# davek44/Glimmer-MG

Hardware: AMD Instinct MI355X
Metric: Mbases/s scored (6-frame IMM) (higher is better)
Workload: dtype f64

## Files before the change

glimmer-mg_amd/csrc/gmg_api.hip:

```cpp

#include "gmg_internal.h"
#include "gmg_scan.h"

#include <ctype.h>
#include <stdarg.h>
#include <stdio.h>
#include <stdlib.h>
#include <string.h>
#include <new>
#include <mutex>
#include <vector>

static thread_local char g_err[512] = "";
static int g_device = -1;

int gmg_set_error(int code, const char *fmt, ...)
{
    va_list ap;
    va_start(ap, fmt);
    vsnprintf(g_err, sizeof g_err, fmt, ap);
    va_end(ap);
    return code;
}

extern "C" const char *gmg_last_error(void) { return g_err; }

long long g_gmg_opt[GMG_OPT_COUNT] = {
     0,  0,  0,  0,  0,  0,
     0,  -1,  0x7ffffffell,  0,  0,
     0,  0,  1,  1,  1,  1,  2,
     -1,  0,  1,  1,  0,  4,  0,  64ll << 20,  0,  0};
static const char *const g_opt_name[GMG_OPT_COUNT] = {
    "seg_plain", "mg_tile", "mg_one_stream", "mg_err_flat", "mg_err_calls", "mg_err_calls_grow", "orfs_exact_path",
    "train_sort_min", "mg_max_entries", "mg_timing", "ingest_timing", "train_timing", "diag", "strings_fused",
    "mg_gene32", "mg_fused", "mg_err_skip", "mg_orfs_events", "mg_err_tile", "mg_err_tile_q", "mg_err_qonly", "mg_err_wave", "mg_err_wave_q", "orfs_walk8", "ingest_scans", "ingest_piece_min", "mg_orfs_bits", "orfs_q_poison"};

static int opt_index(const char *key)
{
    for (int i = 0; key && i < GMG_OPT_COUNT; i++)
        if (strcmp(key, g_opt_name[i]) == 0) return i;
    return -1;
}

extern "C" int gmg_set_option(const char *key, long long value)
{
    const int i = opt_index(key);
    if (i < 0) return gmg_set_error(GMG_EINVAL, "gmg_set_option: unknown option '%s'", key ? key : "(null)");
#ifndef GMG_ABLATIONS
    if (i == GMG_OPT_DIAG && value != 0)
        return gmg_set_error(GMG_EINVAL, "gmg_set_option: the ablation kernels are not in this build (-DGMG_ABLATIONS)");
#endif
    if (i == GMG_OPT_MG_MAX_ENTRIES && (value < 1 || value > 0x7ffffffell))
        return gmg_set_error(GMG_EINVAL, "gmg_set_option: mg_max_entries must be in [1, 2^31 - 2]");
    g_gmg_opt[i] = value;
    return GMG_OK;
}

extern "C" int gmg_get_option(const char *key, long long *value)
{
    const int i = opt_index(key);
    if (i < 0 || !value) return gmg_set_error(GMG_EINVAL, "gmg_get_option: unknown option '%s'", key ? key : "(null)");
    *value = g_gmg_opt[i];
    return GMG_OK;
}

static void options_from_env(void)
{
    for (int i = 0; i < GMG_OPT_COUNT; i++) {
        char name[64] = "GMG_";
        size_t k = 4;
        for (const char *c = g_opt_name[i]; *c && k + 1 < sizeof name; c++) name[k++] = (char)toupper((unsigned char)*c);
        name[k] = 0;
        const char *v = getenv(name);
        if (!v) continue;
        char *end = nullptr;
        long long x = strtoll(v, &end, 10);
        if (end == v) x = 1;
        (void)gmg_set_option(g_opt_name[i], x);
    }
}
extern "C" const char *gmg_version(void) { return "glimmer-mg_amd 0.1 (gfx950)"; }

extern "C" int gmg_device_count(void)
{
    int n = 0;
    if (hipGetDeviceCount(&n) != hipSuccess) return 0;
    return n;
}

extern "C" int gmg_init(int device)
{
    int n = 0;
    hipError_t e = hipGetDeviceCount(&n);
    if (e != hipSuccess || n <= 0)
        return gmg_set_error(GMG_ENODEV, "gmg_init: no HIP device (%s); there is no CPU fallback",
                             e == hipSuccess ? "count = 0" : hipGetErrorString(e));
    if (device < 0 || device >= n)
        return gmg_set_error(GMG_EINVAL, "gmg_init: device %d out of range (have %d)", device, n);
    hipDeviceProp_t prop;
    GMG_HIP(hipGetDeviceProperties(&prop, device));
    if (strncmp(prop.gcnArchName, "gfx950", 6) != 0)
        return gmg_set_error(GMG_ENODEV, "gmg_init: device %d is %s; this library is built for gfx950 only",
                             device, prop.gcnArchName);
    GMG_HIP(hipSetDevice(device));
    if (g_device < 0) options_from_env();
    g_device = device;
    return GMG_OK;
}

int gmg_enter(const char *who)
{
    if (g_device < 0) return gmg_set_error(GMG_ENODEV, "%s: gmg_init() has not succeeded in this process", who);
    int cur = -1;
    if (hipGetDevice(&cur) != hipSuccess || cur != g_device) GMG_HIP(hipSetDevice(g_device));
    return GMG_OK;
}

static int require_init(const char *who) { return gmg_enter(who); }

extern "C" int gmg_synchronize(void *stream)
{
    int rc = gmg_enter("gmg_synchronize");
    if (rc) return rc;
    GMG_HIP(hipStreamSynchronize((hipStream_t)stream));
    return GMG_OK;
}


extern "C" int gmg_base_code(int ch)
{
    switch (tolower(ch & 0xff)) {
    case 'a': return 0;
    case 'c': return 1;
    case 'g': case 'r': case 'd': return 2;
    case 't': case 'w': case 'k': return 3;
    default: return 1;
    }
}

extern "C" uint64_t gmg_packed_words(uint64_t total_bases) { return (total_bases + 15) / 16 + 1; }

static const uint8_t *base_code_table(void)
{
    static const struct Table {
        uint8_t code[256];
        Table() { for (int c = 0; c < 256; c++) code[c] = (uint8_t)gmg_base_code(c); }
    } table;
    return table.code;
}

extern "C" int gmg_pack_bases(const char *ascii, uint64_t n, uint64_t first_base, uint32_t *packed)
{
    if ((!ascii && n) || !packed) return gmg_set_error(GMG_EINVAL, "gmg_pack_bases: NULL argument");
    const uint8_t *code = base_code_table();
    const unsigned char *a = (const unsigned char *)ascii;
    uint64_t i = 0, g = first_base;
    for (; i < n && (g & 15); i++, g++) packed[g >> 4] |= (uint32_t)code[a[i]] << (2 * (g & 15));
    for (; i + 16 <= n; i += 16, g += 16) {
        uint32_t w = 0;
        for (int k = 0; k < 16; k++) w |= (uint32_t)code[a[i + k]] << (2 * k);
        packed[g >> 4] |= w;
    }
    for (; i < n; i++, g++) packed[g >> 4] |= (uint32_t)code[a[i]] << (2 * (g & 15));
    return GMG_OK;
}


static inline int parent_of(int x) { return (x - 1) / 4; }

static int final_row(const int16_t *mip, int n) { return mip[n] == -2 ? parent_of(n) : n; }

static void complete_tree(const int16_t *mip, const float *prob, int D, uint8_t *cshift, float *crow)
{
    std::vector<int> cur(1, 0), nxt;
    size_t lvl_base = 0, lvl_size = 1;
    for (int l = 0; l <= D; l++) {
        if (l < D) nxt.assign(lvl_size * 4, 0);
        for (size_t i = 0; i < lvl_size; i++) {
            int st = cur[i];
            int row = (st >= 0) ? final_row(mip, st) : ~st;
            memcpy(crow + 4 * (lvl_base + i), prob + 4 * (size_t)row, 4 * sizeof(float));
            if (l == D) continue;
            uint8_t sh = 0;
            if (st >= 0 && mip[st] >= 0) {
                sh = (uint8_t)(2 * mip[st]);
                for (int b = 0; b < 4; b++) nxt[4 * i + b] = 4 * st + 1 + b;
            } else {
                for (int b = 0; b < 4; b++) nxt[4 * i + b] = ~row;
            }
            cshift[lvl_base + i] = sh;
        }
        lvl_base += lvl_size;
        lvl_size *= 4;
        cur.swap(nxt);
    }
}

static float dense_entry(const int16_t *mip, const float *prob, int W, int D, uint32_t idx)
{
    int node = 0;
    for (int i = 0; i < D; i++) {
        int pos = mip[node];
        if (pos == -1) break;
        if (pos < -1) { node = parent_of(node); break; }
        node = 4 * node + (int)((idx >> (2 * pos)) & 3) + 1;
    }
    if (mip[node] < -1) node = parent_of(node);
    return prob[4 * (size_t)node + ((idx >> (2 * (W - 1))) & 3)];
}

static float dense_part_entry(const int16_t *mip, const float *prob, int W, int D, int j, uint32_t idx)
{
    int node = 0, start = j - (W - 1);
    for (int i = 0; i < D; i++) {
        int q = start + mip[node];
        if (q < 0) break;
        node = 4 * node + (int)((idx >> (2 * q)) & 3) + 1;
    }
    if (mip[node] == -2) node = parent_of(node);
    return prob[4 * (size_t)node + ((idx >> (2 * j)) & 3)];
}

static size_t align_up(size_t x, size_t a) { return (x + a - 1) / a * a; }

extern "C" int gmg_model_upload(const int16_t *mip, const float *prob4, int W, int D, int P, int N,
                                gmg_model **out)
{
    int rc = require_init("gmg_model_upload");
    if (rc) return rc;
    if (!mip || !prob4 || !out) return gmg_set_error(GMG_EINVAL, "gmg_model_upload: NULL argument");
    if (W < 1 || W > GMG_MAX_MODEL_LEN || D < 0 || D > 12 || P < 1 || N < 1)
        return gmg_set_error(GMG_EBADMODEL, "gmg_model_upload: unsupported shape len=%d depth=%d period=%d nodes=%d",
                             W, D, P, N);
    long need = 0, pw = 1;
    for (int l = 0; l <= D; l++) { need += pw; pw *= 4; }
    if (N < need)
        return gmg_set_error(GMG_EBADMODEL, "gmg_model_upload: num_nodes=%d < %ld needed for depth %d", N, need, D);
    const size_t PN = (size_t)P * N;
    for (size_t i = 0; i < PN; i++)
        if (mip[i] < -2 || mip[i] > W - 1)
            return gmg_set_error(GMG_EBADMODEL, "gmg_model_upload: mut_info_pos %d at slot %zu outside [-2,%d]",
                                 (int)mip[i], i, W - 1);

    const bool fast = (W <= GMG_FAST_MAX_LEN && D <= GMG_FAST_MAX_DEPTH);
    const bool dense = (W <= GMG_DENSE_MAX_LEN);
    const size_t n_internal = (size_t)((pw / 4 - 1) / 3);
    const size_t ctot = (size_t)need;
    const size_t cstride = align_up(n_internal ? n_internal : 1, 16);
    const size_t n_dense = dense ? ((size_t)1 << (2 * W)) : 0;
    const size_t n_part = dense ? (n_dense - 4) / 3 : 0;

    size_t o_mip = 0;
    size_t o_prob = align_up(o_mip + PN, 256);
    size_t o_cshift = align_up(o_prob + PN * 16, 256);
    size_t o_crow = align_up(o_cshift + (fast ? P * cstride : 0), 256);
    size_t o_chalf = align_up(o_crow + (fast ? (size_t)P * ctot * 16 + 16 : 0), 256);
    const size_t n_leaves = (size_t)(pw / 4);
    size_t o_dense = align_up(o_chalf + (fast ? (size_t)P * n_leaves * 16 : 0), 256);
    size_t o_part = align_up(o_dense + (size_t)P * n_dense * 4, 256);
    size_t total = align_up(o_part + (size_t)P * n_part * 4 + 4, 256);

    std::vector<unsigned char> blob(total, 0);
    int8_t *h_mip = (int8_t *)(blob.data() + o_mip);
    for (size_t i = 0; i < PN; i++) h_mip[i] = (int8_t)mip[i];
    memcpy(blob.data() + o_prob, prob4, PN * 16);
    if (fast)
        for (int p = 0; p < P; p++)
            complete_tree(mip + (size_t)p * N, prob4 + 4 * (size_t)p * N, D,
                          blob.data() + o_cshift + p * cstride,
                          (float *)(blob.data() + o_crow) + (size_t)p * ctot * 4);
    if (fast)
        for (int p = 0; p < P; p++) {
            const float *leaf = (const float *)(blob.data() + o_crow) + ((size_t)p * ctot + n_internal) * 4;
            float *half = (float *)(blob.data() + o_chalf) + (size_t)p * n_leaves * 4;
            for (size_t r = 0; r < n_leaves; r++)
                for (int h = 0; h < 2; h++) {
                    half[(h * n_leaves + r) * 2] = leaf[4 * r + 2 * h];
                    half[(h * n_leaves + r) * 2 + 1] = leaf[4 * r + 2 * h + 1];
                }
        }
    if (dense)
        for (int p = 0; p < P; p++) {
            const int16_t *pm = mip + (size_t)p * N;
            const float *pp = prob4 + 4 * (size_t)p * N;
            float *full = (float *)(blob.data() + o_dense) + (size_t)p * n_dense;
            float *part = (float *)(blob.data() + o_part) + (size_t)p * n_part;
            for (uint32_t idx = 0; idx < n_dense; idx++) full[idx] = dense_entry(pm, pp, W, D, idx);
            size_t o = 0;
            for (int j = 0; j < W - 1; j++) {
                uint32_t cnt = 1u << (2 * (j + 1));
                for (uint32_t idx = 0; idx < cnt; idx++) part[o + idx] = dense_part_entry(pm, pp, W, D, j, idx);
                o += cnt;
            }
        }

    gmg_model *m = new (std::nothrow) gmg_model();
    if (!m) return gmg_set_error(GMG_ENOMEM, "gmg_model_upload: out of host memory");
    hipError_t e = hipMalloc(&m->d_blob, total);
    if (e != hipSuccess) { delete m; return gmg_set_error(GMG_ENOMEM, "gmg_model_upload: hipMalloc(%zu): %s", total, hipGetErrorString(e)); }
    e = hipMemcpy(m->d_blob, blob.data(), total, hipMemcpyHostToDevice);
    if (e != hipSuccess) { (void)hipFree(m->d_blob); delete m; return gmg_set_error(GMG_EHIP, "gmg_model_upload: hipMemcpy: %s", hipGetErrorString(e)); }
    m->blob_bytes = total;
    m->min_exp = 255;
    m->max_exp = 0;
    m->odd_values = 0;
    for (size_t i = 0; i < PN * 4; i++) {
        uint32_t b;
        memcpy(&b, &prob4[i], 4);
        const uint32_t ex = (b >> 23) & 0xffu;
        if (mip[i >> 2] == -2) continue;
        if ((b << 1) == 0) continue;
        if ((b >> 31) == 0 || ex == 0 || ex == 255) m->odd_values = 1;
        if ((int)ex < m->min_exp) m->min_exp = (int)ex;
        if ((int)ex > m->max_exp) m->max_exp = (int)ex;
    }
    unsigned char *d = (unsigned char *)m->d_blob;
    m->dev.W = W; m->dev.D = D; m->dev.P = P; m->dev.N = N;
    m->dev.mip = (const int8_t *)(d + o_mip);
    m->dev.prob = (const float *)(d + o_prob);
    m->dev.cshift = fast ? (const uint8_t *)(d + o_cshift) : nullptr;
    m->dev.crow = fast ? (const float *)(d + o_crow) : nullptr;
    m->dev.chalf = fast ? (const float *)(d + o_chalf) : nullptr;
    m->dev.cstride = (int)cstride;
    m->dev.ctot = (int)ctot;
    m->dev.has_fast = fast;
    m->dev.dense = dense ? (const float *)(d + o_dense) : nullptr;
    m->dev.dense_part = dense ? (const float *)(d + o_part) : nullptr;
    m->dev.n_dense_part = (int)n_part;
    m->dev.has_dense = dense;
    *out = m;
    return GMG_OK;
}

extern "C" int gmg_model_free(gmg_model *m)
{
    if (!m) return GMG_OK;
    if (m->d_blob) (void)hipFree(m->d_blob);
    delete m;
    return GMG_OK;
}

extern "C" int gmg_model_info(const gmg_model *m, int *W, int *D, int *P, int *N)
{
    if (!m) return gmg_set_error(GMG_EINVAL, "gmg_model_info: NULL model");
    if (W) *W = m->dev.W;
    if (D) *D = m->dev.D;
    if (P) *P = m->dev.P;
    if (N) *N = m->dev.N;
    return GMG_OK;
}

extern "C" int gmg_null_set_upload(const gmg_model *const *models, int n, gmg_null_set **out)
{
    int rc = require_init("gmg_null_set_upload");
    if (rc) return rc;
    if (!models || n < 1 || !out) return gmg_set_error(GMG_EINVAL, "gmg_null_set_upload: bad argument");
    for (int i = 0; i < n; i++)
        if (!models[i] || !models[i]->dev.has_dense || models[i]->dev.W != 3 || models[i]->dev.P != 3)
            return gmg_set_error(GMG_EBADMODEL, "gmg_null_set_upload: model %d is not a (3,2,3) Build_Indep_WO_Stops model", i);
    gmg_null_set *ns = new (std::nothrow) gmg_null_set();
    if (!ns) return gmg_set_error(GMG_ENOMEM, "gmg_null_set_upload: out of host memory");
    ns->d_tab = nullptr;
    ns->n = n;
    ns->min_exp = 255; ns->max_exp = 0; ns->odd_values = 0;
    for (int i = 0; i < n; i++) {
        if (models[i]->min_exp < ns->min_exp) ns->min_exp = models[i]->min_exp;
        if (models[i]->max_exp > ns->max_exp) ns->max_exp = models[i]->max_exp;
        ns->odd_values |= models[i]->odd_values;
    }
    hipError_t e = hipMalloc((void **)&ns->d_tab, (size_t)n * 252 * sizeof(float));
    for (int i = 0; i < n && e == hipSuccess; i++) {
        e = hipMemcpy(ns->d_tab + (size_t)i * 252, models[i]->dev.dense, 192 * sizeof(float), hipMemcpyDeviceToDevice);
        if (e == hipSuccess) e = hipMemcpy(ns->d_tab + (size_t)i * 252 + 192, models[i]->dev.dense_part, 60 * sizeof(float), hipMemcpyDeviceToDevice);
    }
    if (e != hipSuccess) { gmg_null_set_free(ns); return gmg_set_error(GMG_EHIP, "gmg_null_set_upload: %s", hipGetErrorString(e)); }
    *out = ns;
    return GMG_OK;
}

extern "C" int gmg_null_set_from_tables(const int16_t *mip, const float *prob4, int n, gmg_null_set **out)
{
    int rc = require_init("gmg_null_set_from_tables");
    if (rc) return rc;
    if (!mip || !prob4 || n < 1 || !out) return gmg_set_error(GMG_EINVAL, "gmg_null_set_from_tables: bad argument");
    for (size_t i = 0; i < (size_t)n * 63; i++)
        if (mip[i] < -2 || mip[i] > 2)
            return gmg_set_error(GMG_EBADMODEL, "gmg_null_set_from_tables: mut_info_pos %d in model %zu outside [-2,2]", (int)mip[i], i / 63);
    gmg_null_set *ns = new (std::nothrow) gmg_null_set();
    if (!ns) return gmg_set_error(GMG_ENOMEM, "gmg_null_set_from_tables: out of host memory");
    ns->d_tab = nullptr;
    ns->n = n;
    ns->min_exp = 255; ns->max_exp = 0; ns->odd_values = 0;
    std::vector<float> tab((size_t)n * 252);
    for (int i = 0; i < n; i++)
        for (int p = 0; p < 3; p++) {
            const int16_t *pm = mip + ((size_t)i * 3 + p) * 21;
            const float *pp = prob4 + ((size_t)i * 3 + p) * 21 * 4;
            float *full = tab.data() + (size_t)i * 252 + p * 64, *part = tab.data() + (size_t)i * 252 + 192 + p * 20;
            for (uint32_t idx = 0; idx < 64; idx++) full[idx] = dense_entry(pm, pp, 3, 2, idx);
            size_t o = 0;
            for (int j = 0; j < 2; j++) {
                const uint32_t cnt = 1u << (2 * (j + 1));
                for (uint32_t idx = 0; idx < cnt; idx++) part[o + idx] = dense_part_entry(pm, pp, 3, 2, j, idx);
                o += cnt;
            }
            for (int k = 0; k < 21 * 4; k++) {
                uint32_t b;
                memcpy(&b, pp + k, 4);
// ... 759 lines not shown
```

glimmer-mg_amd/csrc/gmg_frame6.hip:

```cpp

#include "gmg_device.h"
#include <stdlib.h>
#include <vector>

#ifndef GMG_F6_STAMPS
#define GMG_F6_STAMPS 0
#endif
#if GMG_F6_STAMPS
__device__ unsigned long long g_f6_stamps[1024 * 16 * 8];
extern "C" int gmg_debug_f6_stamps(unsigned long long *out, int n)
{
    return hipMemcpyFromSymbol(out, HIP_SYMBOL(g_f6_stamps), (size_t)n * 8) == hipSuccess ? 0 : -1;
}
#define F6_STAMP(i) do { const unsigned long long now_ = __builtin_readcyclecounter(); st_acc[i] += now_ - st_prev; st_prev = now_; } while (0)
#else
#define F6_STAMP(i) do { } while (0)
#endif

struct Frame6Args {
    GmgDevModel gene, nul;
    const uint32_t *packed;
    const uint64_t *off;
    const uint32_t *tile_read;
    uint64_t total, n_reads;
// ... 380 lines not shown
                        const double nf = s_nf[__builtin_amdgcn_ubfe(mt, mb + 4 + 2 * b, 6)];
                        const double nr = s_nr[__builtin_amdgcn_ubfe(mt, mb + 2 * b, 6)];
                        v[2 * b] = (double)gf - nf;
                        v[2 * b + 1] = (double)gr - nr;
                    }
                }
                const uint64_t chunk = MULTI ? round_chunk0 + (uint64_t)k : chunk0 + (uint64_t)(j0 + k) * chunk_step;
                if (SUM) {
                    sum_chunk((uint32_t)k, v);
                } else if (GENE_ONLY) {
                    float *gf = a.out_gene + (uint64_t)(STRINGS ? 1 : ftype) * a.gstride + chunk * SPAN;
                    float *gr = a.out_gene + (uint64_t)(STRINGS ? 0 : 3 + ftype) * a.gstride + chunk * SPAN;
                    if (PAIR) {
                        typedef float f2 __attribute__((ext_vector_type(2)));
                        const f2 x0 = {(float)v[0], (float)v[2]}, x1 = {(float)v[1], (float)v[3]};
                        __builtin_nontemporal_store(x0, (f2 *)(gf + lane_off));
                        __builtin_nontemporal_store(x1, (f2 *)(gr + lane_off));
                    } else {
                        gf[lane_off] = (float)v[0]; gf[lane_off + 1] = (float)v[2];
                        gr[lane_off] = (float)v[1]; gr[lane_off + 1] = (float)v[3];
                    }
                } else if (DIAG & 1) {
                    if (v[0] + v[1] + v[2] + v[3] == 1.2345e300) a.out[lane_off] = v[0];
                } else {
                    double *pf = out_f + chunk * SPAN, *pr = out_r + chunk * SPAN;
                    if (PAIR) {
                        typedef double d2 __attribute__((ext_vector_type(2)));
                        const d2 x0 = {v[0], v[2]}, x1 = {v[1], v[3]};
                        __builtin_nontemporal_store(x0, (d2 *)(pf + lane_off));
                        __builtin_nontemporal_store(x1, (d2 *)(pr + lane_off));
                    } else {
                        __builtin_nontemporal_store(v[0], pf + lane_off);
                        __builtin_nontemporal_store(v[2], pf + lane_off + 1);
                        __builtin_nontemporal_store(v[1], pr + lane_off);
                        __builtin_nontemporal_store(v[3], pr + lane_off + 1);
                    }
                }
            }
        }
        if (SUM) {
            __syncthreads();
            round_flush();
        }
        F6_STAMP(4);
    }
#if GMG_F6_STAMPS
    if ((threadIdx.x & 63u) == 0 && blockIdx.x < 1024)
        for (int i = 0; i < 8; i++) g_f6_stamps[(blockIdx.x * 16 + (threadIdx.x >> 6)) * 8 + i] = st_acc[i];
#endif
}


__device__ __forceinline__ void f6_generic_range(const Frame6Args &a, const GmgDevModel &gene, uint64_t first, uint64_t count,
                                                 uint64_t i0, uint64_t n_lanes)
{
    for (uint64_t i = i0; i < count; i += n_lanes) {
        const uint64_t g = first + i;
        uint64_t r = a.tile_read[g / GMG_TILE];
        uint64_t r_end = a.off[r + 1];
        while (g >= r_end) { r++; r_end = a.off[r + 1]; }
        const uint64_t r_off = a.off[r];
        const int L = (int)(r_end - r_off);
        const int p = (int)(g - r_off);
        DevBuf bf = dev_make_buf(a.packed, r_off, 0, (uint32_t)L, GMG_REVERSED);
        DevBuf br = dev_make_buf(a.packed, r_off, 0, (uint32_t)L, GMG_COMPLEMENTED);
        for (int f = 0; f < 3; f++) {
            if (a.out_gene) {
                a.out_gene[(uint64_t)f * a.gstride + g] = dev_score(gene, bf, L - 1 - p, f);
                a.out_gene[(uint64_t)(3 + f) * a.gstride + g] = dev_score(gene, br, p, f);
                continue;
            }
            a.out[(uint64_t)f * a.stride + g] =
                (double)dev_score(gene, bf, L - 1 - p, f) - (double)dev_score(a.nul, bf, L - 1 - p, f);
            a.out[(uint64_t)(3 + f) * a.stride + g] =
                (double)dev_score(gene, br, p, f) - (double)dev_score(a.nul, br, p, f);
        }
    }
}
__device__ __forceinline__ void f6_generic_range(const Frame6Args &a, uint64_t i0, uint64_t n_lanes)
{
    f6_generic_range(a, a.gene, a.first, a.count, i0, n_lanes);
}

template <int DT, int U, bool GENE = false, bool MULTI = false>
__global__ __launch_bounds__(256) void k_frame6p(Frame6Args a)
{
    extern __shared__ __attribute__((aligned(16))) uint8_t s_shift[];
    if (MULTI) {
        if (blockIdx.x < 8 * a.n_ranges) {
            const F6Range rg = a.ranges[blockIdx.x / 8];
            f6_generic_range(a, a.gmodels[rg.group], rg.first, rg.count, (uint64_t)(blockIdx.x % 8) * blockDim.x + threadIdx.x, (uint64_t)8 * blockDim.x);
            return;
        }
    } else if (blockIdx.x >= a.p_blocks) {
        f6_generic_range(a, (uint64_t)(blockIdx.x - a.p_blocks) * blockDim.x + threadIdx.x, (uint64_t)(gridDim.x - a.p_blocks) * blockDim.x);
        return;
    }
    const int cstride = a.gene.cstride;
    const float *crow = a.gene.crow;
    int ctot = a.gene.ctot;
    if (!MULTI) {
        for (int i = threadIdx.x * 16; i < 3 * cstride; i += 256 * 16)
            *(uint4 *)(s_shift + i) = *(const uint4 *)(a.gene.cshift + i);
        __syncthreads();
    }

    const int W = a.gene.W, D = DT > 0 ? DT : a.gene.D, Wn = a.nul.W;
    const uint32_t Z = 2u * (uint32_t)(W - 1);
    const uint32_t ctx_mask = (W >= 16) ? 0xffffffffu : ((1u << (2 * W)) - 1u);
    const int n_dense = 1 << (2 * Wn);
    const int n_part = a.nul.n_dense_part;
    const uint32_t z = threadIdx.x & 31u;
    const bool rev_buf = z >= (uint32_t)(W - 1);
    const int j = rev_buf ? (int)z - (W - 1) : (int)z;
    const int thr2 = 2 * ((W - 1) - j);
    const uint64_t reads_per_pass = (uint64_t)a.p_blocks * (256 / 32);

    const float *ntab = (j >= Wn - 1) ? a.nul.dense : a.nul.dense_part;
    const int nstride = (j >= Wn - 1) ? n_dense : n_part;

    const uint32_t pb = MULTI ? blockIdx.x - 8 * a.n_ranges : blockIdx.x;
    const uint64_t share_lo = MULTI ? a.n_reads * pb / a.p_blocks : 0, share_hi = MULTI ? a.n_reads * (pb + 1) / a.p_blocks : a.n_reads;
    uint32_t grp = 0;
    if (MULTI) {
        uint32_t lo = 0, hi = a.n_groups;
        while (hi - lo > 1) { const uint32_t mid = (lo + hi) >> 1; if (a.group_read[mid] <= share_lo) lo = mid; else hi = mid; }
        grp = lo;
    }
    for (uint64_t part_lo = share_lo; part_lo < share_hi;) {
    uint64_t part_hi = share_hi;
    if (MULTI) {
        while (a.group_read[grp + 1] <= part_lo) grp++;
        if (a.group_read[grp + 1] < part_hi) part_hi = a.group_read[grp + 1];
        const GmgDevModel &gm = a.gmodels[grp];
        __syncthreads();
        for (int i = threadIdx.x * 16; i < 3 * cstride; i += 256 * 16)
            *(uint4 *)(s_shift + i) = *(const uint4 *)(gm.cshift + i);
        __syncthreads();
        crow = gm.crow;
        ctot = gm.ctot;
    }
    const uint64_t r_step = MULTI ? 256 / 32 : reads_per_pass;
    for (uint64_t r0 = (MULTI ? part_lo : (uint64_t)blockIdx.x * (256 / 32)) + (threadIdx.x >> 5); r0 < part_hi; r0 += U * r_step) {
        bool live[U];
        uint64_t g[U];
        uint32_t C[U];
#pragma unroll
        for (int u = 0; u < U; u++) {
            const uint64_t r = r0 + u * r_step;
            const bool in = r < part_hi;
            const uint64_t rq = in ? r : part_hi - 1;
            const uint64_t r_off = a.off[rq];
            const int L = (int)(a.off[rq + 1] - r_off);
            live[u] = in && z < Z && j < L;
            const int p = rev_buf ? L - 1 - j : j;
            g[u] = r_off + (uint64_t)(live[u] ? p : 0);
        }
#pragma unroll
        for (int u = 0; u < U; u++) {
            const uint64_t x = dev_window_bits(a.packed, (int64_t)g[u] - (W - 1));
            C[u] = rev_buf ? dev_reverse_fields((uint32_t)(x >> (2 * (W - 1))) & ctx_mask, W)
                           : (((uint32_t)x & ctx_mask) ^ ctx_mask);
        }
        uint32_t idx[U][3], node[U][3];
#pragma unroll
        for (int u = 0; u < U; u++)
#pragma unroll
            for (int f = 0; f < 3; f++) { idx[u][f] = 0; node[u][f] = 0xffffffffu; }
        uint32_t lvl = 0, width = 1;
#pragma unroll
        for (int l = 0; l < (DT > 0 ? DT : 12); l++) {
            if (DT == 0 && l >= D) break;
#pragma unroll
            for (int u = 0; u < U; u++)
#pragma unroll
                for (int f = 0; f < 3; f++) {
                    const uint32_t sh = s_shift[f * cstride + lvl + idx[u][f]];
                    if (node[u][f] == 0xffffffffu && (int)sh < thr2) node[u][f] = lvl + idx[u][f];
                    idx[u][f] = (idx[u][f] << 2) + ((C[u] >> sh) & 3u);
                }
            lvl += width;
            width <<= 2;
        }
        float gv[U][3], nv[U][3];
#pragma unroll
        for (int u = 0; u < U; u++) {
            const uint32_t pred = (C[u] >> (2 * (W - 1))) & 3u;
            const uint32_t nslot = (j >= Wn - 1) ? (C[u] >> (2 * (W - Wn)))
                                                 : (C[u] >> (2 * (W - 1 - j))) + (((1u << (2 * (j + 1))) - 4u) / 3u);
#pragma unroll
            for (int f = 0; f < 3; f++) {
                if (node[u][f] == 0xffffffffu) node[u][f] = lvl + idx[u][f];
                gv[u][f] = crow[((size_t)f * ctot + node[u][f]) * 4 + pred];
                nv[u][f] = GENE ? 0.0f : ntab[(size_t)f * nstride + nslot];
            }
        }
#pragma unroll
        for (int u = 0; u < U; u++)
            if (live[u])
#pragma unroll
                for (int f = 0; f < 3; f++) {
                    if (GENE)
                        a.out_gene[(uint64_t)((rev_buf ? 0 : 3) + f) * a.gstride + g[u]] = gv[u][f];
                    else
                        __builtin_nontemporal_store((double)gv[u][f] - (double)nv[u][f],
                                                    a.out + (uint64_t)((rev_buf ? 0 : 3) + f) * a.stride + g[u]);
                }
    }
    part_lo = part_hi;
    }
}

__global__ __launch_bounds__(256) void k_frame6_generic(Frame6Args a)
{
    f6_generic_range(a, (uint64_t)blockIdx.x * blockDim.x + threadIdx.x, (uint64_t)gridDim.x * blockDim.x);
}

static int launch_generic(Frame6Args a, uint64_t first, uint64_t count, hipStream_t s)
{
    if (count == 0) return GMG_OK;
    a.first = first;
    a.count = count;
    const uint64_t blocks = (count + 255) / 256;
    const unsigned grid = (unsigned)(blocks < 256 * 16 ? blocks : 256 * 16);
    hipLaunchKernelGGL(k_frame6_generic, dim3(grid), dim3(256), 0, s, a);
    GMG_HIP(hipGetLastError());
    return GMG_OK;
}

int gmg_launch_frame6(const gmg_model *gene, const gmg_model *nul, const gmg_reads *reads, double *d_out,
                      hipStream_t s)
{
    return gmg_launch_frame6_strided(gene, nul, reads, d_out, reads->total_bases, s);
}

int gmg_launch_frame6_strided(const gmg_model *gene, const gmg_model *nul, const gmg_reads *reads, double *d_out,
                              uint64_t stride, hipStream_t s)
{
    Frame6Args a;
    a.gene = gene->dev;
    a.nul = nul->dev;
    a.packed = reads->d_packed;
    a.off = reads->d_off;
    a.tile_read = reads->d_tile_read;
    a.total = reads->total_bases;
    a.n_reads = reads->n_reads;
    a.first = 0;
    a.count = 0;
    a.out = d_out;
    a.stride = stride;
    a.out_gene = nullptr;
    a.gstride = 0;
    a.str_sums = nullptr;
    a.uniform_len = 0;
    a.str_sums = nullptr;
    a.uniform_len = 0;

    const bool fast = gene->dev.has_fast && gene->dev.D == 7 && nul->dev.has_dense && nul->dev.W == 3 &&
                      gene->dev.W >= 3 && gene->dev.W <= 15;
    if (!fast) return launch_generic(a, 0, a.total, s);

    constexpr int BLOCK = 1024, DT = 7;
    constexpr uint32_t SPAN = 2 * BLOCK;
    constexpr int KR = 16;
    const uint64_t n_chunks = a.total / SPAN;
    const int diag = (int)gmg_opt(GMG_OPT_DIAG);
    const bool pair = (a.stride & 1) == 0;
    if (n_chunks > 0) {
        int dev = 0, n_cu = 256;
        GMG_HIP(hipGetDevice(&dev));
        GMG_HIP(hipDeviceGetAttribute(&n_cu, hipDeviceAttributeMultiprocessorCount, dev));
        unsigned nworkers = (unsigned)(n_cu / 3);
        if (nworkers < 1) nworkers = 1;
        if (nworkers > n_chunks) nworkers = (unsigned)n_chunks;
        const unsigned grid = 3 * nworkers;
        const size_t lds = ((size_t)1 << (2 * DT)) * 8;
#define GMG_LAUNCH_F6T(DIAG_, P_)                                                                       \
    do {                                                                                                \
        GMG_HIP(hipFuncSetAttribute((const void *)k_frame6t<BLOCK, DT, KR, DIAG_, P_, false>,           \
                                    hipFuncAttributeMaxDynamicSharedMemorySize, (int)lds));             \
        hipLaunchKernelGGL((k_frame6t<BLOCK, DT, KR, DIAG_, P_, false>), dim3(grid), dim3(BLOCK), lds, s, a); \
    } while (0)
        if (diag == 0) { if (pair) GMG_LAUNCH_F6T(0, true); else GMG_LAUNCH_F6T(0, false); }
#ifdef GMG_ABLATIONS
        else if (diag == 1 && pair) GMG_LAUNCH_F6T(1, true);
        else if (diag == 2 && pair) GMG_LAUNCH_F6T(2, true);
        else if (diag == 3 && pair) GMG_LAUNCH_F6T(3, true);
#endif
        else return gmg_set_error(GMG_EINVAL, "the ablation kernel diag=%d is not in this build", diag);
#undef GMG_LAUNCH_F6T
        GMG_HIP(hipGetLastError());
    }
    if (a.n_reads > 0) {
        const uint64_t blocks = (a.n_reads + 7) / 8;
        const unsigned grid = (unsigned)(blocks < 256 * 8 ? blocks : 256 * 8);
        const size_t lds_p = (size_t)3 * a.gene.cstride;
        a.first = n_chunks * SPAN;
        a.count = a.total - n_chunks * SPAN;
        a.p_blocks = grid;
        const unsigned tail_blocks = (unsigned)((a.count + 255) / 256);
        hipLaunchKernelGGL((k_frame6p<7, 4>), dim3(grid + tail_blocks), dim3(256), lds_p, s, a);
        GMG_HIP(hipGetLastError());
    }
    return GMG_OK;
}

static int gene6_impl(const gmg_model *gene, const gmg_reads *reads, float *d_gene, uint64_t gstride, bool full, hipStream_t s)
{
    if (!(gene->dev.has_fast && gene->dev.D == 7 && gene->dev.W >= 3 && gene->dev.W <= 15 && gene->dev.P >= 3))
        return GMG_EBADMODEL;
    Frame6Args a;
    a.gene = gene->dev;
    a.nul = gene->dev;
    a.packed = reads->d_packed;
    a.off = reads->d_off;
    a.tile_read = reads->d_tile_read;
    a.total = reads->total_bases;
    a.n_reads = reads->n_reads;
    a.first = 0;
    a.count = 0;
    a.out = nullptr;
    a.stride = 0;
    a.out_gene = d_gene;
    a.gstride = gstride;
    a.str_sums = nullptr;
    a.uniform_len = 0;
    constexpr int BLOCK = 1024, DT = 7, KR = 16;
    constexpr uint32_t SPAN = 2 * BLOCK;
    const uint64_t n_chunks = a.total / SPAN;
    if (n_chunks > 0) {
        int dev = 0, n_cu = 256;
        GMG_HIP(hipGetDevice(&dev));
        GMG_HIP(hipDeviceGetAttribute(&n_cu, hipDeviceAttributeMultiprocessorCount, dev));
        unsigned nworkers = (unsigned)(n_cu / 3);
        if (nworkers < 1) nworkers = 1;
        if (nworkers > n_chunks) nworkers = (unsigned)n_chunks;
        const unsigned grid = 3 * nworkers;
        const size_t lds = ((size_t)1 << (2 * DT)) * 8;
        if ((gstride & 1) == 0) {
            GMG_HIP(hipFuncSetAttribute((const void *)k_frame6t<BLOCK, DT, KR, 0, true, true>,
                                        hipFuncAttributeMaxDynamicSharedMemorySize, (int)lds));
            hipLaunchKernelGGL((k_frame6t<BLOCK, DT, KR, 0, true, true>), dim3(grid), dim3(BLOCK), lds, s, a);
        } else {
            GMG_HIP(hipFuncSetAttribute((const void *)k_frame6t<BLOCK, DT, KR, 0, false, true>,
                                        hipFuncAttributeMaxDynamicSharedMemorySize, (int)lds));
            hipLaunchKernelGGL((k_frame6t<BLOCK, DT, KR, 0, false, true>), dim3(grid), dim3(BLOCK), lds, s, a);
        }
        GMG_HIP(hipGetLastError());
    }
    if (!full) return launch_generic(a, n_chunks * SPAN, a.total - n_chunks * SPAN, s);
    if (a.n_reads > 0) {
        const uint64_t blocks = (a.n_reads + 7) / 8;
        const unsigned grid = (unsigned)(blocks < 256 * 8 ? blocks : 256 * 8);
        const size_t lds_p = (size_t)3 * a.gene.cstride;
        a.first = n_chunks * SPAN;
        a.count = a.total - n_chunks * SPAN;
        a.p_blocks = grid;
        const unsigned tail_blocks = (unsigned)((a.count + 255) / 256);
        hipLaunchKernelGGL((k_frame6p<7, 4, true>), dim3(grid + tail_blocks), dim3(256), lds_p, s, a);
        GMG_HIP(hipGetLastError());
    }
    return GMG_OK;
}

int gmg_launch_gene6(const gmg_model *gene, const gmg_reads *reads, float *d_gene, hipStream_t s)
{
    return gene6_impl(gene, reads, d_gene, reads->total_bases, false, s);
}

int gmg_launch_gene6_full(const gmg_model *gene, const gmg_reads *reads, float *d_gene, uint64_t gstride, hipStream_t s)
{
    return gene6_impl(gene, reads, d_gene, gstride, true, s);
}

__global__ void k_f6_gather_u64(const uint64_t *src, const uint64_t *idx, uint32_t n, uint64_t *dst)
{
    const uint32_t i = blockIdx.x * blockDim.x + threadIdx.x;
    if (i < n) dst[i] = src[idx[i]];
}

int gmg_launch_gene6_groups(const gmg_model *const *models, const uint64_t *group_read, int n_groups, const gmg_reads *reads,
                            float *d_gene, uint64_t gstride, hipStream_t s)
{
    if (!models || !group_read || n_groups < 1 || n_groups > F6_MAX_GROUPS || group_read[0] != 0 || group_read[n_groups] != reads->n_reads)
        return gmg_set_error(GMG_EINVAL, "gmg_launch_gene6_groups: bad group list");
    for (int g = 0; g < n_groups; g++)
        if (!models[g] || group_read[g + 1] < group_read[g] || models[g]->dev.P < 3)
            return gmg_set_error(GMG_EINVAL, "gmg_launch_gene6_groups: group %d has no periodicity-3 model or an inverted read range", g);
    if (reads->total_bases == 0) return GMG_OK;
    constexpr int BLOCK = 1024, DT = 7, KR = 16;
    constexpr uint32_t SPAN = 2 * BLOCK;

    std::vector<uint64_t> base(n_groups + 1);
    {
        uint64_t *d_idx = nullptr, *d_val = nullptr;
        GMG_HIP(gmg_pool_alloc((void **)&d_idx, (size_t)(n_groups + 1) * 8));
        hipError_t e = gmg_pool_alloc((void **)&d_val, (size_t)(n_groups + 1) * 8);
        if (e != hipSuccess) {
            gmg_pool_release(d_idx);
            return gmg_set_error(e == hipErrorOutOfMemory ? GMG_ENOMEM : GMG_EHIP, "gmg_launch_gene6_groups: %s", hipGetErrorString(e));
        }
        e = hipMemcpyAsync(d_idx, group_read, (size_t)(n_groups + 1) * 8, hipMemcpyHostToDevice, s);
        if (e == hipSuccess) {
            hipLaunchKernelGGL(k_f6_gather_u64, dim3((n_groups + 256) / 256), dim3(256), 0, s, reads->d_off, d_idx, (uint32_t)(n_groups + 1), d_val);
            e = hipMemcpyAsync(base.data(), d_val, (size_t)(n_groups + 1) * 8, hipMemcpyDeviceToHost, s);
        }
        if (e == hipSuccess) e = hipStreamSynchronize(s);
        gmg_pool_release(d_idx);
        gmg_pool_release(d_val);
        if (e != hipSuccess) return gmg_set_error(GMG_EHIP, "gmg_launch_gene6_groups: %s", hipGetErrorString(e));
    }

    Frame6Args a;
    a.gene = models[0]->dev;
    a.nul = models[0]->dev;
    a.packed = reads->d_packed;
    a.off = reads->d_off;
    a.tile_read = reads->d_tile_read;
    a.total = reads->total_bases;
    a.n_reads = reads->n_reads;
    a.first = 0;
    a.count = 0;
    a.p_blocks = 0;
    a.out = nullptr;
    a.stride = 0;
    a.out_gene = d_gene;
    a.gstride = gstride;
    a.str_sums = nullptr;
    a.uniform_len = 0;

    bool fast = true;
    for (int g = 0; g < n_groups && fast; g++) {
        const GmgDevModel &m = models[g]->dev;
        fast = m.has_fast && m.D == 7 && m.W >= 3 && m.W <= 15 && m.W == models[0]->dev.W && m.cstride == models[0]->dev.cstride;
    }
    if (!fast) {
        for (int g = 0; g < n_groups; g++) {
            a.gene = models[g]->dev;
            const int rc = launch_generic(a, base[g], base[g + 1] - base[g], s);
            if (rc) return rc;
        }
// ... 168 lines not shown
```

glimmer-mg_amd/csrc/gmg_internal.h:

```cpp
#ifndef GMG_INTERNAL_H
#define GMG_INTERNAL_H

#include <hip/hip_runtime.h>
#include <stdint.h>
#include <vector>
#include "../../include/gmg.h"

#define GMG_MAX_MODEL_LEN 32
#define GMG_FAST_MAX_LEN 16
#define GMG_FAST_MAX_DEPTH 8
#define GMG_DENSE_MAX_LEN 6
#define GMG_TILE 1024
#define GMG_GUARD_WORDS 320

struct GmgDevModel {
    int W, D, P, N;
    const int8_t *mip;
    const float *prob;
    const uint8_t *cshift;
    const float *crow;
    const float *chalf;
    int cstride;
    int ctot;
    int has_fast;
    const float *dense;
    const float *dense_part;
    int n_dense_part;
    int has_dense;
};

struct gmg_model {
    int min_exp, max_exp, odd_values;
    GmgDevModel dev;
    void *d_blob;
    size_t blob_bytes;
};

struct gmg_reads {
    const uint32_t *d_packed;
    const uint64_t *d_off;
    uint32_t *d_tile_read;
    uint64_t n_reads;
    uint64_t total_bases;
    uint64_t n_tiles;
    uint64_t n_words;
    void *d_packed_alloc;
    int owns_off;
    int uniform_len;
    uint64_t max_len, min_len;
    uint64_t n_over_512;
};

struct gmg_null_set {
    float *d_tab;
    int n;
    int min_exp, max_exp, odd_values;
};

struct gmg_segments {
    gmg_segment *d_segs;
    uint64_t *d_out_off;
    uint64_t n;
    uint64_t total_len;
    uint64_t min_len;
};

int gmg_set_error(int code, const char *fmt, ...);
int gmg_enter(const char *who);
#define GMG_HIP(call)                                                                         \
    do {                                                                                      \
        hipError_t e_ = (call);                                                               \
        if (e_ != hipSuccess)                                                                 \
            return gmg_set_error(GMG_EHIP, "%s failed: %s (%s:%d)", #call, hipGetErrorString(e_), \
                                 __FILE__, __LINE__);                                         \
    } while (0)

enum GmgOpt {
    GMG_OPT_SEG_PLAIN,
    GMG_OPT_MG_TILE,
    GMG_OPT_MG_ONE_STREAM,
    GMG_OPT_MG_ERR_FLAT,
    GMG_OPT_MG_ERR_CALLS,
    GMG_OPT_MG_ERR_CALLS_GROW,
    GMG_OPT_ORFS_EXACT_PATH,
    GMG_OPT_TRAIN_SORT_MIN,
    GMG_OPT_MG_MAX_ENTRIES,
    GMG_OPT_MG_TIMING,
    GMG_OPT_INGEST_TIMING,
    GMG_OPT_TRAIN_TIMING,
    GMG_OPT_DIAG,
    GMG_OPT_STRINGS_FUSED,
    GMG_OPT_MG_GENE32,
    GMG_OPT_MG_FUSED,
    GMG_OPT_MG_ERR_SKIP,
    GMG_OPT_MG_ORFS_EVENTS,
    GMG_OPT_MG_ERR_TILE,
    GMG_OPT_MG_ERR_TILE_Q,
    GMG_OPT_MG_ERR_QONLY,
    GMG_OPT_MG_ERR_WAVE,
    GMG_OPT_MG_ERR_WAVE_Q,
    GMG_OPT_ORFS_WALK8,
    GMG_OPT_INGEST_SCANS,
    GMG_OPT_INGEST_PIECE_MIN,
    GMG_OPT_MG_ORFS_BITS,
    GMG_OPT_ORFS_Q_POISON,
    GMG_OPT_COUNT
};
extern long long g_gmg_opt[GMG_OPT_COUNT];
static inline long long gmg_opt(int k) { return g_gmg_opt[k]; }

void gmg_ingest_trim(void);
hipError_t gmg_pool_alloc(void **out, size_t bytes);
void gmg_pool_release(void *p);
void gmg_pool_release_after(void *p, hipStream_t s);

struct __attribute__((visibility("hidden"))) GmgScratch {
    enum Wait { NONE, STREAM, DEVICE };
    Wait wait = NONE;
    hipStream_t st = nullptr;
    std::vector<void *> v;
    GmgScratch() {}
    GmgScratch(const GmgScratch &) = delete;
    GmgScratch &operator=(const GmgScratch &) = delete;
    ~GmgScratch()
    {
        if (wait == STREAM) (void)hipStreamSynchronize(st);
        else if (wait == DEVICE) (void)hipDeviceSynchronize();
        for (void *p : v) gmg_pool_release(p);
    }
    template <class T> hipError_t alloc(T **p, size_t bytes)
    {
        const hipError_t e = gmg_pool_alloc((void **)p, bytes);
        if (e == hipSuccess) v.push_back(*p);
        return e;
    }
    template <class T> void detach(T *p)
    {
        for (size_t k = 0; k < v.size(); k++)
            if (v[k] == (void *)p) { v[k] = v.back(); v.pop_back(); return; }
    }
    template <class T> void release(T *&p)
    {
        if (!p) return;
        detach(p);
        gmg_pool_release(p);
        p = nullptr;
    }
};

int gmg_launch_tile_read(const uint64_t *d_off, uint64_t n_reads, uint64_t n_tiles, uint32_t *d_tile_read,
                         hipStream_t s);
int gmg_launch_frame6(const gmg_model *gene, const gmg_model *nul, const gmg_reads *reads, double *d_out,
                      hipStream_t s);
int gmg_launch_frame6_strided(const gmg_model *gene, const gmg_model *nul, const gmg_reads *reads, double *d_out,
                              uint64_t stride, hipStream_t s);
int gmg_launch_gene6(const gmg_model *gene, const gmg_reads *reads, float *d_gene, hipStream_t s);
int gmg_launch_gene6_full(const gmg_model *gene, const gmg_reads *reads, float *d_gene, uint64_t gstride, hipStream_t s);
int gmg_launch_gene6_groups(const gmg_model *const *models, const uint64_t *group_read, int n_groups, const gmg_reads *reads,
                            float *d_gene, uint64_t gstride, hipStream_t s);
int gmg_launch_strings(const gmg_model *m, const gmg_reads *reads, float *d_vals, uint64_t *tail_start, hipStream_t s);
int gmg_launch_strings_sum(const gmg_model *m, const gmg_reads *reads, double *d_sums, uint64_t *tail_start, hipStream_t s);
int gmg_launch_seg_frame(const gmg_model *m, const gmg_reads *r, const gmg_segments *sg, int frame,
                         double *d_out, hipStream_t s);
int gmg_launch_seg_cum(const gmg_model *m, const gmg_reads *r, const gmg_segments *sg, int frame0,
                       double *d_out, double *d_sums, hipStream_t s);
int gmg_launch_seg_partial(const gmg_model *m, const gmg_reads *r, const gmg_segments *sg, int frame,
                           double *d_out, hipStream_t s);
int gmg_launch_all_frame(const gmg_model *m, const gmg_reads *r, const gmg_segments *sg,
                         const uint32_t *d_prefix, const int32_t *d_frame, double *d_af, hipStream_t s);
int gmg_launch_fixed(const gmg_fixed_model *m, const gmg_reads *r, const gmg_segments *sg, int lo, int hi,
                     double *d_out, hipStream_t s);
int gmg_launch_windows(const gmg_model *m, const uint8_t *d_windows, const int32_t *d_frames, uint64_t n,
                       float *d_dist4, double *d_prob, hipStream_t s);

#endif
```

Measured before the change: 100,700.

## Add per-read heads kernel for frame6 scoring of read-edge positions

Adds a new kernel, k_frame6h, which gives the first and last W-1 positions of each read (the heads) to one lane per read. Each lane walks the context tree for these positions and stages the resulting crow offsets and null slots in LDS. The wave then redistributes the work so that loads and stores are coalesced. A host-side check verifies that the tree's stop levels allow this per-level walk, and the path is enabled by default through a new f6_heads option. It also adds diagnostic ablation variants. The cost it targets is divergent per-position work on read edges in the old path, and in exchange it uses more LDS, adds code complexity and relies on new correctness assumptions.

```diff
diff --git a/glimmer-mg_amd/csrc/gmg_api.hip b/glimmer-mg_amd/csrc/gmg_api.hip
--- a/glimmer-mg_amd/csrc/gmg_api.hip
+++ b/glimmer-mg_amd/csrc/gmg_api.hip
@@ -29,11 +29,12 @@
      0,  0,  0,  0,  0,  0,
      0,  -1,  0x7ffffffell,  0,  0,
      0,  0,  1,  1,  1,  1,  2,
-     -1,  0,  1,  1,  0,  4,  0,  64ll << 20,  0,  0};
+     -1,  0,  1,  1,  0,  4,  0,  64ll << 20,  0,  0,
+     1};
 static const char *const g_opt_name[GMG_OPT_COUNT] = {
     "seg_plain", "mg_tile", "mg_one_stream", "mg_err_flat", "mg_err_calls", "mg_err_calls_grow", "orfs_exact_path",
     "train_sort_min", "mg_max_entries", "mg_timing", "ingest_timing", "train_timing", "diag", "strings_fused",
-    "mg_gene32", "mg_fused", "mg_err_skip", "mg_orfs_events", "mg_err_tile", "mg_err_tile_q", "mg_err_qonly", "mg_err_wave", "mg_err_wave_q", "orfs_walk8", "ingest_scans", "ingest_piece_min", "mg_orfs_bits", "orfs_q_poison"};
+    "mg_gene32", "mg_fused", "mg_err_skip", "mg_orfs_events", "mg_err_tile", "mg_err_tile_q", "mg_err_qonly", "mg_err_wave", "mg_err_wave_q", "orfs_walk8", "ingest_scans", "ingest_piece_min", "mg_orfs_bits", "orfs_q_poison", "f6_heads"};
 
 static int opt_index(const char *key)
 {
@@ -194,6 +195,25 @@
         lvl_size *= 4;
         cur.swap(nxt);
     }
+}
+
+static bool heads_stop_by_level(const uint8_t *cshift, int W, int D)
+{
+    std::vector<uint8_t> up, cur;
+    size_t lvl_base = 0, lvl_size = 1;
+    for (int l = 0; l < D && l < W - 1; l++) {
+        cur.resize(lvl_size);
+        for (size_t i = 0; i < lvl_size; i++) {
+            uint8_t m = cshift[lvl_base + i];
+            if (l > 0 && up[i >> 2] < m) m = up[i >> 2];
+            if ((int)m >= 2 * (W - 1 - l)) return false;
+            cur[i] = m;
+        }
+        lvl_base += lvl_size;
+        lvl_size *= 4;
+        up.swap(cur);
+    }
+    return true;
 }
 
 static float dense_entry(const int16_t *mip, const float *prob, int W, int D, uint32_t idx)
@@ -324,6 +344,9 @@
     m->dev.cstride = (int)cstride;
     m->dev.ctot = (int)ctot;
     m->dev.has_fast = fast;
+    m->dev.heads_by_level = fast;
+    for (int p = 0; p < P && m->dev.heads_by_level; p++)
+        m->dev.heads_by_level = heads_stop_by_level(blob.data() + o_cshift + p * cstride, W, D);
     m->dev.dense = dense ? (const float *)(d + o_dense) : nullptr;
     m->dev.dense_part = dense ? (const float *)(d + o_part) : nullptr;
     m->dev.n_dense_part = (int)n_part;
diff --git a/glimmer-mg_amd/csrc/gmg_frame6.hip b/glimmer-mg_amd/csrc/gmg_frame6.hip
--- a/glimmer-mg_amd/csrc/gmg_frame6.hip
+++ b/glimmer-mg_amd/csrc/gmg_frame6.hip
@@ -486,7 +486,7 @@
     f6_generic_range(a, a.gene, a.first, a.count, i0, n_lanes);
 }
 
-template <int DT, int U, bool GENE = false, bool MULTI = false>
+template <int DT, int U, bool GENE = false, bool MULTI = false, int PDIAG = 0>
 __global__ __launch_bounds__(256) void k_frame6p(Frame6Args a)
 {
     extern __shared__ __attribute__((aligned(16))) uint8_t s_shift[];
@@ -575,6 +575,7 @@
 #pragma unroll
         for (int l = 0; l < (DT > 0 ? DT : 12); l++) {
             if (DT == 0 && l >= D) break;
+            if (PDIAG == 3) break;
 #pragma unroll
             for (int u = 0; u < U; u++)
 #pragma unroll
@@ -595,6 +596,12 @@
 #pragma unroll
             for (int f = 0; f < 3; f++) {
                 if (node[u][f] == 0xffffffffu) node[u][f] = lvl + idx[u][f];
+                if (PDIAG == 3) node[u][f] = (C[u] & 0x3fffu) + (uint32_t)f;
+                if (PDIAG == 2) {
+                    gv[u][f] = __uint_as_float(0x3f800000u | (node[u][f] * 4u + pred));
+                    nv[u][f] = (float)nslot;
+                    continue;
+                }
                 gv[u][f] = crow[((size_t)f * ctot + node[u][f]) * 4 + pred];
                 nv[u][f] = GENE ? 0.0f : ntab[(size_t)f * nstride + nslot];
             }
@@ -606,6 +613,8 @@
                 for (int f = 0; f < 3; f++) {
                     if (GENE)
                         a.out_gene[(uint64_t)((rev_buf ? 0 : 3) + f) * a.gstride + g[u]] = gv[u][f];
+                    else if (PDIAG == 1 && (double)gv[u][f] - (double)nv[u][f] != 1.2345e300)
+                        continue;
                     else
                         __builtin_nontemporal_store((double)gv[u][f] - (double)nv[u][f],
                                                     a.out + (uint64_t)((rev_buf ? 0 : 3) + f) * a.stride + g[u]);
@@ -615,9 +624,191 @@
     }
 }
 
+constexpr int F6H_BLOCK = 256;
+constexpr int F6H_MAXP = 14;
+constexpr uint32_t F6H_NULL = 256;
+constexpr uint32_t f6h_top_floats(int topl) { return topl > 0 ? ((3u * 4u * (uint32_t)f6_level_base(topl) + 3u) & ~3u) : 0u; }
+static size_t f6h_lds_bytes(const GmgDevModel &gene, int topl)
+{
+    return (size_t)3 * gene.cstride + F6H_NULL * 4 + f6h_top_floats(topl) * 4 + (size_t)(F6H_BLOCK / 64) * 3 * 64 * (gene.W - 1) * 4;
+}
+
+template <int DT, int WM1C, bool GENE, int TOPL = 0, int HDIAG = 0>
+__global__ __launch_bounds__(F6H_BLOCK) void k_frame6h(Frame6Args a)
+{
+    constexpr uint32_t CTOT = f6_level_base(DT + 1);
+    static_assert(3 * CTOT * 4 <= (1u << 18), "a crow offset must fit the 18 bits of a staged word");
+    extern __shared__ __attribute__((aligned(16))) uint8_t s_h[];
+    if (blockIdx.x >= a.p_blocks) {
+        f6_generic_range(a, (uint64_t)(blockIdx.x - a.p_blocks) * blockDim.x + threadIdx.x, (uint64_t)(gridDim.x - a.p_blocks) * blockDim.x);
+        return;
+    }
+    const uint32_t hblock = blockIdx.x;
+    constexpr uint32_t TOPN = TOPL > 0 ? f6_level_base(TOPL) : 0;
+    const uint32_t cstride = (uint32_t)a.gene.cstride;
+    const uint32_t wm1 = WM1C > 0 ? (uint32_t)WM1C : (uint32_t)(a.gene.W - 1);
+    const uint8_t *s_shift = s_h;
+    float *s_null = (float *)(s_h + 3 * cstride);
+    float *s_top = s_null + F6H_NULL;
+    uint32_t *s_stage = (uint32_t *)(s_top + f6h_top_floats(TOPL)) + (threadIdx.x >> 6) * (3 * 64 * wm1);
+    for (uint32_t i = threadIdx.x * 16; i < 3 * cstride; i += F6H_BLOCK * 16)
+        *(uint4 *)(s_h + i) = *(const uint4 *)(a.gene.cshift + i);
+    if (!GENE && threadIdx.x < 3 * 64 + 3 * 20)
+        s_null[threadIdx.x] = threadIdx.x < 192 ? a.nul.dense[threadIdx.x] : a.nul.dense_part[threadIdx.x - 192];
+    if (TOPL > 0)
+        for (uint32_t i = threadIdx.x; i < 3 * TOPN; i += F6H_BLOCK)
+            *(float4 *)(s_top + 4 * i) = *(const float4 *)(a.gene.crow + ((size_t)(i / (TOPN ? TOPN : 1)) * CTOT + i % (TOPN ? TOPN : 1)) * 4);
+    __syncthreads();
+
+    const uint32_t lane = threadIdx.x & 63u;
+    const uint32_t ctx_mask = (1u << (2 * (wm1 + 1))) - 1u;
+    const uint32_t inv = (65536u + wm1 - 1u) / wm1;
+    uint32_t sh0[3];
+#pragma unroll
+    for (int f = 0; f < 3; f++) sh0[f] = __builtin_amdgcn_readfirstlane((uint32_t)s_shift[f * cstride]);
+    const uint32_t ulen = a.uniform_len;
+    const float *crow = a.gene.crow;
+
+    for (uint64_t r0 = (uint64_t)hblock * F6H_BLOCK + (threadIdx.x & ~63u); r0 < a.n_reads; r0 += (uint64_t)a.p_blocks * F6H_BLOCK) {
+        const uint64_t r = r0 + lane;
+        uint64_t off_r;
+        uint32_t L;
+        if (ulen) {
+            off_r = (r < a.n_reads ? r : a.n_reads) * ulen;
+            L = r < a.n_reads ? ulen : 0u;
+        } else {
+            off_r = a.off[r < a.n_reads ? r : a.n_reads];
+            L = (uint32_t)(a.off[r < a.n_reads ? r + 1 : a.n_reads] - off_r);
+        }
+        const uint32_t first16 = (uint32_t)dev_window_bits(a.packed, (int64_t)off_r);
+        const uint32_t last16 = (uint32_t)dev_window_bits(a.packed, (int64_t)(off_r + L) - 16);
+        const uint32_t Bc = ~first16, Br = dev_reverse_fields(last16, 16);
+
+#pragma unroll
+        for (int b = 0; b < 2; b++) {
+            const uint32_t B = b ? Br : Bc;
+#pragma unroll
+            for (int j = 0; j < F6H_MAXP; j++) {
+                if (WM1C > 0 ? j >= WM1C : (uint32_t)j >= wm1) break;
+                const uint32_t thr2 = 2u * (wm1 - (uint32_t)j);
+                const uint32_t Cw = (B << thr2) & ctx_mask;
+                const uint32_t pred = (B >> (2 * j)) & 3u;
+                const uint32_t nslot = j >= 2 ? ((B >> (2 * (j >= 2 ? j - 2 : 0))) & 63u)
+                                              : 192u + (B & ((1u << (2 * (j + 1))) - 1u)) + (j ? 4u : 0u);
+                const uint32_t nstep = j >= 2 ? 64u : 20u;
+                const uint32_t k = b ? wm1 - 1u - (uint32_t)j : (uint32_t)j;
+                const int nl = j < DT ? j : DT;
+#pragma unroll
+                for (int f = 0; f < 3; f++) {
+                    uint32_t idx = 0, node = 0;
+                    bool open = true;
+#pragma unroll
+                    for (int l = 0; l < nl; l++) {
+                        const uint32_t sh = l == 0 ? sh0[f] : (uint32_t)s_shift[f * cstride + f6_level_base(l) + idx];
+                        const bool stop = open && sh < thr2;
+                        node = stop ? (uint32_t)f6_level_base(l) + idx : node;
+                        open = open && !stop;
+                        idx = (idx << 2) | __builtin_amdgcn_ubfe(Cw, sh, 2);
+                    }
+                    if (open) node = (uint32_t)f6_level_base(nl) + idx;
+                    s_stage[(uint32_t)f * 64u * wm1 + lane * wm1 + k] =
+                        (((uint32_t)f * CTOT + node) * 4u + pred) | (GENE ? 0u : (nslot + (uint32_t)f * nstep) << 18);
+                }
+            }
+            wcs_sync();
+            float gv[F6H_MAXP][3];
+            uint64_t g[F6H_MAXP];
+            bool live[F6H_MAXP];
+#pragma unroll
+            for (int i = 0; i < F6H_MAXP; i++) {
+                if (WM1C > 0 ? i >= WM1C : (uint32_t)i >= wm1) break;
+                const uint32_t t = lane + 64u * (uint32_t)i;
+                const uint32_t q = (t * inv) >> 16, k = t - q * wm1;
+                const uint32_t j = b ? wm1 - 1u - k : k;
+                uint64_t off_q;
+                uint32_t L_q;
+                if (ulen) {
+                    off_q = (r0 + q) * ulen;
+                    L_q = r0 + q < a.n_reads ? ulen : 0u;
+                } else {
+                    const uint32_t lo = (uint32_t)__builtin_amdgcn_ds_bpermute((int)(q << 2), (int)(uint32_t)off_r);
+                    const uint32_t hi = (uint32_t)__builtin_amdgcn_ds_bpermute((int)(q << 2), (int)(uint32_t)(off_r >> 32));
+                    off_q = (uint64_t)hi << 32 | lo;
+                    L_q = (uint32_t)__builtin_amdgcn_ds_bpermute((int)(q << 2), (int)L);
+                }
+                live[i] = j < L_q;
+                g[i] = off_q + (b ? L_q - 1u - j : j);
+#pragma unroll
+                for (int f = 0; f < 3; f++) {
+                    const uint32_t x = s_stage[(uint32_t)f * 64u * wm1 + t] & 0x3ffffu, top = x - (uint32_t)f * CTOT * 4u;
+                    gv[i][f] = 0.0f;
+                    if (HDIAG == 2) gv[i][f] = __uint_as_float(0x3f800000u | x);
+                    else if (TOPL > 0 && top < TOPN * 4u) gv[i][f] = s_top[(uint32_t)f * TOPN * 4u + top];
+                    else if (live[i]) gv[i][f] = crow[x];
+                }
+            }
+#pragma unroll
+            for (int i = 0; i < F6H_MAXP; i++) {
+                if (WM1C > 0 ? i >= WM1C : (uint32_t)i >= wm1) break;
+                if (!live[i]) continue;
+#pragma unroll
+                for (int f = 0; f < 3; f++) {
+                    if (GENE) {
+                        a.out_gene[(uint64_t)((b ? 0 : 3) + f) * a.gstride + g[i]] = gv[i][f];
+                        continue;
+                    }
+                    const double v = (double)gv[i][f] - (double)s_null[s_stage[(uint32_t)f * 64u * wm1 + lane + 64u * (uint32_t)i] >> 18];
+                    if (HDIAG == 1 && v != 1.2345e300) continue;
+                    __builtin_nontemporal_store(v, a.out + (uint64_t)((b ? 0 : 3) + f) * a.stride + g[i]);
+                }
+            }
+            wcs_sync();
+        }
+    }
+}
+
 __global__ __launch_bounds__(256) void k_frame6_generic(Frame6Args a)
 {
     f6_generic_range(a, (uint64_t)blockIdx.x * blockDim.x + threadIdx.x, (uint64_t)gridDim.x * blockDim.x);
+}
+
+static bool f6_heads_per_read(const GmgDevModel &gene)
+{
+    const long long diag = gmg_opt(GMG_OPT_DIAG);
+    return gmg_opt(GMG_OPT_F6_HEADS) != 0 && gene.heads_by_level && (diag == 0 || diag == 7 || diag == 11);
+}
+static unsigned f6h_blocks(uint64_t n_reads)
+{
+    const uint64_t blocks = (n_reads + F6H_BLOCK - 1) / F6H_BLOCK;
+    return (unsigned)(blocks < (1u << 20) ? blocks : (1u << 20));
+}
+
+template <bool GENE>
+static int launch_heads_per_read(Frame6Args a, const gmg_reads *reads, unsigned tail_blocks, hipStream_t s)
+{
+    a.uniform_len = reads->uniform_len > 0 ? (uint32_t)reads->uniform_len : 0u;
+    a.p_blocks = f6h_blocks(a.n_reads);
+    const dim3 grid(a.p_blocks + tail_blocks), block(F6H_BLOCK);
+    const long long mode = gmg_opt(GMG_OPT_F6_HEADS), diag = gmg_opt(GMG_OPT_DIAG);
+    (void)diag;
+#define GMG_LAUNCH_F6H(WM1C_, TOPL_, HD_)                                                                                   \
+    do {                                                                                                                    \
+        const size_t lds = f6h_lds_bytes(a.gene, TOPL_);                                                                    \
+        if (lds > 64 * 1024)                                                                                                \
+            GMG_HIP(hipFuncSetAttribute((const void *)k_frame6h<7, WM1C_, GENE, TOPL_, HD_>, hipFuncAttributeMaxDynamicSharedMemorySize, (int)lds)); \
+        hipLaunchKernelGGL((k_frame6h<7, WM1C_, GENE, TOPL_, HD_>), grid, block, lds, s, a);                                \
+    } while (0)
+    if (a.gene.W != 12 || mode == 2) GMG_LAUNCH_F6H(0, 0, 0);
+#ifdef GMG_ABLATIONS
+    else if (diag == 7 && !GENE) GMG_LAUNCH_F6H(11, 0, 1);
+    else if (diag == 11 && !GENE) GMG_LAUNCH_F6H(11, 0, 2);
+#endif
+    else if (mode == 3) GMG_LAUNCH_F6H(11, 5, 0);
+    else if (mode == 4) GMG_LAUNCH_F6H(0, 5, 0);
+    else GMG_LAUNCH_F6H(11, 0, 0);
+#undef GMG_LAUNCH_F6H
+    GMG_HIP(hipGetLastError());
+    return GMG_OK;
 }
 
 static int launch_generic(Frame6Args a, uint64_t first, uint64_t count, hipStream_t s)
@@ -687,6 +878,7 @@
     } while (0)
         if (diag == 0) { if (pair) GMG_LAUNCH_F6T(0, true); else GMG_LAUNCH_F6T(0, false); }
 #ifdef GMG_ABLATIONS
+        else if (diag >= 4 && diag <= 11 && pair) GMG_LAUNCH_F6T(0, true);
         else if (diag == 1 && pair) GMG_LAUNCH_F6T(1, true);
         else if (diag == 2 && pair) GMG_LAUNCH_F6T(2, true);
         else if (diag == 3 && pair) GMG_LAUNCH_F6T(3, true);
@@ -703,6 +895,13 @@
         a.count = a.total - n_chunks * SPAN;
         a.p_blocks = grid;
         const unsigned tail_blocks = (unsigned)((a.count + 255) / 256);
+        if (f6_heads_per_read(a.gene)) return launch_heads_per_read<false>(a, reads, tail_blocks, s);
+#ifdef GMG_ABLATIONS
+        if (diag == 4) hipLaunchKernelGGL((k_frame6p<7, 4, false, false, 1>), dim3(grid + tail_blocks), dim3(256), lds_p, s, a);
+        else if (diag == 5) hipLaunchKernelGGL((k_frame6p<7, 4, false, false, 2>), dim3(grid + tail_blocks), dim3(256), lds_p, s, a);
+        else if (diag == 6) hipLaunchKernelGGL((k_frame6p<7, 4, false, false, 3>), dim3(grid + tail_blocks), dim3(256), lds_p, s, a);
+        else
+#endif
         hipLaunchKernelGGL((k_frame6p<7, 4>), dim3(grid + tail_blocks), dim3(256), lds_p, s, a);
         GMG_HIP(hipGetLastError());
     }
@@ -761,6 +960,7 @@
         a.count = a.total - n_chunks * SPAN;
         a.p_blocks = grid;
         const unsigned tail_blocks = (unsigned)((a.count + 255) / 256);
+        if (f6_heads_per_read(a.gene)) return launch_heads_per_read<true>(a, reads, tail_blocks, s);
         hipLaunchKernelGGL((k_frame6p<7, 4, true>), dim3(grid + tail_blocks), dim3(256), lds_p, s, a);
         GMG_HIP(hipGetLastError());
     }
diff --git a/glimmer-mg_amd/csrc/gmg_internal.h b/glimmer-mg_amd/csrc/gmg_internal.h
--- a/glimmer-mg_amd/csrc/gmg_internal.h
+++ b/glimmer-mg_amd/csrc/gmg_internal.h
@@ -23,6 +23,7 @@
     int cstride;
     int ctot;
     int has_fast;
+    int heads_by_level;
     const float *dense;
     const float *dense_part;
     int n_dense_part;
@@ -104,6 +105,7 @@
     GMG_OPT_INGEST_PIECE_MIN,
     GMG_OPT_MG_ORFS_BITS,
     GMG_OPT_ORFS_Q_POISON,
+    GMG_OPT_F6_HEADS,
     GMG_OPT_COUNT
 };
 extern long long g_gmg_opt[GMG_OPT_COUNT];
```

After: 100000. About the same (-0.7%).
